# lawfuyang/ToyRenderer

Hardware: AMD Instinct MI355X
Metric: Gmeshlets/s culled (whole node), 100M meshlets (higher is better)
Workload: dtype f32

## Files before the change

toyrenderer_amd/csrc/k_basepass_as.hip:

```cpp
#include <algorithm>
#include <cstdlib>
#include <string>
#include <type_traits>

#if defined(TR_STAMPS) || defined(TR_COUNT_SLOW) || defined(TR_COUNT_PATHS)
__device__ unsigned long long g_stampSums[8];
#define g_pathCount (g_stampSums + 4)
#endif
#include <atomic>
#include <memory>
#include <mutex>
#include <unordered_map>

#include "cull_math.hip.h"
#include "instance_cache.hip.h"
#include "meshlet_exact.hip.h"
#include "trhip_internal.h"

using namespace interop;

namespace
{

constexpr uint32_t kBlock = 256;
// ... 115 lines not shown
#ifdef TR_STAMPS
#define TR_STAMP(i) do { unsigned long long _t = __builtin_amdgcn_s_memtime(); __builtin_amdgcn_s_waitcnt(0xC07F); stampSum[i] += _t - stampLast; stampLast = _t; } while (0)
#else
#define TR_STAMP(i) do {} while (0)
#endif

#ifndef TR_LK_POLICY_ID
#define TR_LK_POLICY_ID 0
#endif
#if TR_LK_POLICY_ID == 0
#define TR_LK_POLICY ""
#elif TR_LK_POLICY_ID == 1
#define TR_LK_POLICY " sc0"
#elif TR_LK_POLICY_ID == 2
#define TR_LK_POLICY " sc1"
#elif TR_LK_POLICY_ID == 3
#define TR_LK_POLICY " sc0 sc1"
#elif TR_LK_POLICY_ID == 4
#define TR_LK_POLICY " nt"
#else
#define TR_LK_POLICY " sc1 nt"
#endif
#ifndef TR_CULL_WAVES_PER_EU
#define TR_CULL_WAVES_PER_EU 5
#endif
template <bool FRUSTUM, bool OCCLUSION, bool CONE, bool TABLE>
__global__ __launch_bounds__(kCullBlock, TR_CULL_WAVES_PER_EU) void meshletCullKernel(MeshletCullArgs a)
{
#ifdef TR_STAMPS
    unsigned long long stampSum[8] = {0, 0, 0, 0, 0, 0, 0, 0};
    unsigned long long stampLast = __builtin_amdgcn_s_memtime();
    __builtin_amdgcn_s_waitcnt(0xC07F);
#endif
    __shared__ RecordInfo s_recAll[kCullWaves][kCullBatch + 2 * kRingSlots];
    __shared__ uint32_t s_gIdxAll[kCullWaves][kCullBatch];
    __shared__ uint32_t s_quadOff[16];
    __shared__ uint4 s_mipTab[17];
    __shared__ float s_coneTab[cm::kConeTabEntries];
    constexpr bool kDeferred = OCCLUSION && TABLE;
    __shared__ uint2 s_mipBand[kDeferred ? 17 : 1];
    __shared__ uint32_t s_defAll[kCullWaves][kDeferred ? kDefStage * kDefWords : 1u];
    __shared__ __attribute__((aligned(8))) uint32_t s_maskAll[kCullWaves][kCullBatch + 2];
    __shared__ __attribute__((aligned(16))) char s_ring[kCullWaves][kRingSlots][kSlotBytes];

    const uint32_t G = groupCount(a);
    const uint32_t tid = threadIdx.x, lane = tid & 63u, wave = tid >> 6;
    const uint32_t half = lane >> 5, sub = lane & 31u;
    if (a.listGroups && blockIdx.x == 0 && tid == 0) a.listGroups[0] = G;
    const cm::M43 V = cm::loadM43(a.k.m_WorldToView);
    const cm::M43P VP = cm::packM43(V);
    const cm::M33P VR = cm::rot(VP);
    const float coneSlack = cm::coneSlackFactor(V);
    if (!TABLE && G <= gridDim.x * (2u * kCullWaves) * a.shortPassRounds) {
        for (uint32_t g = (blockIdx.x * kCullWaves + wave) * 2u + half; g < G; g += gridDim.x * kCullWaves * 2u) {
            const bool vis = exactMeshletVisible<FRUSTUM, OCCLUSION, CONE>(a, VP, VR, g, sub);
            const unsigned long long b = __ballot(vis);
            if (sub == 0) a.visMask[g] = (uint32_t)(half ? b >> 32 : b);
        }
        return;
    }
    RecordInfo* s_rec = s_recAll[wave];
    uint32_t* s_gIdx = s_gIdxAll[wave];

    if (tid < 16) s_quadOff[tid] = a.hzb.mipOffset[tid];
    if (TABLE && tid >= 1 && tid <= 16) {
        const uint32_t mip = tid - 1u < a.hzb.mips ? tid - 1u : 0u;
        const uint32_t mw = (a.hzb.width >> mip) ? (a.hzb.width >> mip) : 1u, mh = (a.hzb.height >> mip) ? (a.hzb.height >> mip) : 1u;
        s_mipTab[tid] = make_uint4(a.quad.offset[mip], ((mw >> 3) + 1u) * 64u, __float_as_uint(0.5f * (float)mw), __float_as_uint(0.5f * (float)mh));
    }
    if (kDeferred && tid >= 1 && tid <= 16) { const uint32_t d = cm::projMipDelta(a.bands, tid); s_mipBand[tid] = make_uint2(d, 2u * d); }
    const bool nearInRange = a.k.m_NearPlane >= 0x1p-20f && a.k.m_NearPlane <= 0x1p20f;
    if (CONE) for (uint32_t i = tid; i < cm::kConeTabEntries; i += kCullBlock) s_coneTab[i] = cm::coneTableEntry(i);
    if (lane < 2 * kRingSlots) { s_recAll[wave][kCullBatch + lane].first = 0; s_recAll[wave][kCullBatch + lane].lastOff = 0; }
    uint32_t* s_def = s_defAll[wave];
    uint32_t* s_mask = s_maskAll[wave];
    __syncthreads();

    const bool usePerm = a.permHeader != nullptr && a.permHeader[0] == 1u && a.permHeader[1] == G;
#ifndef TR_TEAM_ALL
    const uint32_t teamWaves = kCullWaves, waveInTeam = wave, team = blockIdx.x, teams = gridDim.x;
#else
    const uint32_t teamWaves = gridDim.x * kCullWaves, waveInTeam = blockIdx.x * kCullWaves + wave, team = 0u, teams = 1u;
#endif
    const uint32_t superSize = teamWaves * kCullBatch;
    const uint32_t numSuper = (G + superSize - 1) / superSize;
    auto loadEntry = [&](uint32_t sb_) -> uint4 {
#ifdef TR_BLOCKED_MAP
        const uint64_t e64 = (uint64_t)sb_ * superSize + waveInTeam * kCullBatch + lane;
#else
        const uint64_t e64 = (uint64_t)sb_ * superSize + (lane >> 1) * 2 * teamWaves + 2 * waveInTeam + (lane & 1);
#endif
        if (lane >= kCullBatch || sb_ >= numSuper || e64 >= G) return make_uint4(0xFFFFFFFFu, 0u, 0u, 0u);
        const uint32_t e = (uint32_t)e64;
        if (usePerm) return a.perm[e];
        const MeshletAmplificationData rec = a.records[e];
        return make_uint4(e, rec.m_InstanceConstIdx, rec.m_MeshLOD, rec.m_MeshletGroupOffset);
    };
#ifndef TR_NO_SPLIT_TAIL
    const uint32_t fullRounds = numSuper / teams, left = numSuper - fullRounds * teams;
    uint32_t piecesPer = 1u, stepsPer = kCullSteps;
    if (left) {
        const uint32_t k = std::min(teams / left, kCullSteps / kRingSlots);
        if (k > 1u) {
            stepsPer = ((kCullSteps + k - 1u) / k + kRingSlots - 1u) / kRingSlots * kRingSlots;
            piecesPer = (kCullSteps + stepsPer - 1u) / stepsPer;
        }
// ... 1003 lines not shown
    }
    if (rc != TRHIP_OK) return rc;
    a.meshlets = (const MeshletData*)meshlets->ptr;
    TRHIP_REQUIRE(meshlets->byteSize >= sizeof(MeshletData), "%s: empty meshlet buffer", ctx.shaderName);
    rc = meshlets->cullStream.allocate(meshlets->dev, meshletStreamBytes(meshlets->byteSize / sizeof(MeshletData)));
    if (rc != TRHIP_OK) return rc;
    a.stream = meshletStreamLayout(meshlets->cullStream.ptr, meshlets->byteSize / sizeof(MeshletData));
    a.records = (const MeshletAmplificationData*)records->ptr;
    a.dispatchArgs = (const uint32_t*)((const char*)ctx.argsBuffer->ptr + ctx.argsOffset);
    a.argsWords = (ctx.argsBuffer->byteSize - ctx.argsOffset) >= 16 ? 4u : 3u;
    const uint64_t cap = records->byteSize / sizeof(MeshletAmplificationData);
    a.recordCapacity = cap > 0xFFFFFFFFull ? 0xFFFFFFFFu : (uint32_t)cap;
    TRHIP_REQUIRE(a.recordCapacity <= (1u << 27), "%s: more than 2^27 records cannot be encoded as (g<<5)|lane", ctx.shaderName);
    TRHIP_REQUIRE(visMask->byteSize / 4 >= a.recordCapacity, "%s: visMask holds %llu groups, records buffer %u", ctx.shaderName,
                  (unsigned long long)(visMask->byteSize / 4), a.recordCapacity);
    a.numMeshlets = meshlets->byteSize / sizeof(MeshletData);
    TRHIP_REQUIRE(a.numMeshlets <= (1ull << 32), "%s: more than 2^32 meshlets (m_MeshletDataBufferIdx is 32 bits wide)", ctx.shaderName);
    a.visMask = (uint32_t*)visMask->ptr;
    a.visibleList = (uint32_t*)visList->ptr;
    const uint64_t lcap = visList->byteSize / 4;
    a.listCapacity = lcap > 0xFFFFFFFFull ? 0xFFFFFFFFu : (uint32_t)lcap;
    a.drawArgs = (uint32_t*)drawArgs->ptr;
    if (records->order.ptr && records->order.bytes >= 256 + (uint64_t)a.recordCapacity * 16) {
        a.permHeader = (const uint32_t*)records->order.ptr;
        a.perm = (const uint4*)(a.permHeader + 64);
    }
    rc = trhip::instanceCacheEnsure(instances);
    if (rc != TRHIP_OK) return rc;
    a.numInstances = (uint32_t)(instances->byteSize / sizeof(BasePassInstanceConstants));
    a.cache = instanceCacheLayout(instances->cullCache.ptr, a.numInstances);
    a.maxBatches = (a.recordCapacity + kBatch - 1) / kBatch;
    a.batchSum = (uint32_t*)(a.recordCapacity >= (1u << 19) ? ctx.scratchSide((size_t)a.maxBatches * 4)
                                                            : ctx.scratch((size_t)a.maxBatches * 4));
    TRHIP_REQUIRE(a.batchSum, "%s: scratch allocation failed", ctx.shaderName);
    {
        const size_t supers = (a.maxBatches >> kSuperShift) + 1u;
        a.superSum = (uint32_t*)(a.recordCapacity >= (1u << 19) ? ctx.scratchSide(supers * 4) : ctx.scratch(supers * 4));
        TRHIP_REQUIRE(a.superSum, "%s: scratch allocation failed", ctx.shaderName);
    }

    const uint32_t blocksPerCU = TR_CULL_WAVES_PER_EU;
    uint32_t grid = ctx.computeUnits() * blocksPerCU;
    const uint32_t needBlocks = (a.recordCapacity + kCullBatch * kCullWaves - 1) / (kCullBatch * kCullWaves);
    if (grid > needBlocks) grid = needBlocks;
    if (grid == 0) grid = 1;
    rc = visMask->listCount.allocate(visMask->dev, 256);
    if (rc != TRHIP_OK) return rc;
    a.listGroups = (uint32_t*)visMask->listCount.ptr;
    ctx.cl->use(a.listGroups, ctx.cl->ops.size(), true);
    if (useTable) a.bands = cm::projBands(k->m_P00, k->m_P11, hzb->width, hzb->height);
    static const bool noShortPass = getenv("TRHIP_NO_SHORT_PASS") != nullptr;
    a.shortPassRounds = noShortPass ? 0u : kShortPassRounds;
    const uint32_t flags = k->m_CullingFlags & 7u;
    trhip_texture_t* quadOwner = useTable ? hzb : nullptr;
    const bool table = useTable;
    if (quadOwner) ctx.cl->use(quadOwner->quad.ptr, ctx.cl->ops.size(), false);
    ctx.emit("cull", [a, grid, flags, quadOwner, table, instances, meshData, meshlets](hipStream_t s) {
        if ((const void*)a.meshlets != meshlets->ptr)
            return trhip::fail(TRHIP_ERR_STATE, "basepass_AS_Main: the meshlet buffer was bound to other memory after this command list was recorded: record it again");
        {
            int crc = trhip::instanceCacheLaunchBuild(instances, meshData, s);
            if (crc != TRHIP_OK) return crc;
            crc = meshletStreamLaunchBuild(meshlets, s);
            if (crc != TRHIP_OK) return crc;
        }
        if (quadOwner) {
            int brc = trhip::hzbQuadLaunchBuild(quadOwner, s);
            if (brc != TRHIP_OK) return brc;
        }
        switch (flags) {
        case 0: launchCull<false, false, false>(a, grid, table, s); break;
        case 1: launchCull<true, false, false>(a, grid, table, s); break;
        case 2: launchCull<false, true, false>(a, grid, table, s); break;
        case 3: launchCull<true, true, false>(a, grid, table, s); break;
        case 4: launchCull<false, false, true>(a, grid, table, s); break;
        case 5: launchCull<true, false, true>(a, grid, table, s); break;
        case 6: launchCull<false, true, true>(a, grid, table, s); break;
        default: launchCull<true, true, true>(a, grid, table, s); break;
        }
        return trhip::launchStatus("meshletCullKernel"); });
    emitListBuild(ctx, a, "", a.recordCapacity >= (1u << 19), ctx.argsBuffer->ptr);
    if (ctx.cl->openStats)
        return trhip::statsEmitAS(ctx, a, meshlets, records, instances, meshData, a.recordCapacity >= (1u << 19));
    return TRHIP_OK;
}

int recordPackShard(trhip::DispatchCtx& ctx)
{
    const uint32_t* push = (const uint32_t*)ctx.constants(0, 8);
    trhip_buffer_t* slot = ctx.buffer(TRHIP_BIND_STRUCTURED_UAV, 0);
    trhip_buffer_t* state = ctx.buffer(TRHIP_BIND_STRUCTURED_UAV, 1);
    TRHIP_REQUIRE(push && slot && state, "%s: needs push constants {slotGroups, slotRuns}, UAV u0 (shard slot) and UAV u1 (state words, zeroed once)", ctx.shaderName);
    ShardPackArgs a;
    memset(&a, 0, sizeof a);
    a.slotGroups = push[0];
    a.slotRuns = push[1];
    const uint64_t slotWords = (uint64_t)kSlotHeaderWords + 4ull * a.slotRuns + a.slotGroups;
    TRHIP_REQUIRE(slot->byteSize >= slotWords * 4, "%s: shard slot buffer smaller than 16 + 4 * %u + %u words", ctx.shaderName, a.slotRuns, a.slotGroups);
    const uint64_t maxTiles = (uint64_t)a.slotGroups / kPackTile + kMaxPassSlots + 1u;
    TRHIP_REQUIRE(maxTiles < (1u << 30) && state->byteSize >= maxTiles * 16u, "%s: state buffer u1 smaller than %llu bytes", ctx.shaderName, (unsigned long long)(maxTiles * 16u));
    TRHIP_REQUIRE(((uintptr_t)slot->ptr & 15u) == 0 && ((uintptr_t)state->ptr & 7u) == 0, "%s: u0 / u1 not 16 / 8-byte aligned", ctx.shaderName);
    a.slot = (uint32_t*)slot->ptr;
    a.maxTiles = (uint32_t)maxTiles;
    unsigned long long* halves = (unsigned long long*)state->ptr;
    for (uint32_t s = 0; s < kMaxPassSlots; ++s) {
        trhip_buffer_t* rec = ctx.buffer(TRHIP_BIND_STRUCTURED_SRV, 4 * s);
// ... 122 lines not shown
```

toyrenderer_amd/csrc/k_gpuculling.hip:

```cpp
#include "cull_math.hip.h"
#include "hzb_quad.hip.h"
#include "instance_cache.hip.h"
#include "trhip_internal.h"

using namespace interop;

namespace
{

constexpr uint32_t kBlock = 256;
constexpr uint32_t kWordSubmit = 1u << 30;
constexpr uint32_t kWordLate = 1u << 31;
constexpr uint32_t kGroupMask = (1u << 27) - 1u;

struct InstanceCullArgs
{
    GPUCullingPassConstants k;
    const BasePassInstanceConstants* instances;
    const uint32_t* ids;
    const MeshData* meshData;
    cm::Hzb hzb;
    MeshletAmplificationData* records;
    uint32_t* dispatchArgs;
    uint32_t* lateCount;
    uint32_t* lateIds;
    const uint32_t* indirectArgs;
    InstanceCullCache cache;
    uint32_t numInstances;
    const uint32_t* shardLate;
    uint32_t directThreads;
    uint32_t maxGroups;
    uint32_t argsWords;
    uint32_t* word;
    uint32_t* localOff;
    uint32_t* blockGroups;
    uint64_t* blockLateSubmit;
    uint32_t* bases;
    uint32_t numBlocks;
    uint32_t* tileHist;
    uint32_t* tileTotal;
    uint16_t* tileOf;
    uint2* lodSel;
    uint32_t* permHeader;
    uint4* perm;
    uint32_t permCapacity;
    uint32_t* lateArgsOut;
    unsigned long long* fusedStatus;
    uint32_t* fusedTicket;
};

struct QuadShare { bool stale = false; };
struct EarlyCullNote { InstanceCullArgs a; size_t scanOp; bool fused; trhip_texture_t* quadOwner = nullptr; std::shared_ptr<QuadShare> share; };

__global__ __launch_bounds__(256) void instanceCacheKernel(const BasePassInstanceConstants* instances, uint32_t n,
                                                           const MeshData* meshData, uint32_t numMeshes, InstanceCullCache c)
// ... 367 lines not shown
        const bool emitRec = submit && !dropped;
        const uint32_t id = emitRec ? a.ids[t] : 0u;
        if (emitRec) {
            struct __attribute__((packed, aligned(4))) Quad { uint32_t x, y, z, w; };
            uint32_t* dst = reinterpret_cast<uint32_t*>(a.records + off);
            uint32_t i = 0;
            for (; i + 4u <= groups; i += 4u) {
                const uint32_t o = i * kNumThreadsPerWave;
                *reinterpret_cast<Quad*>(dst + 3u * i) = Quad{ id, lod, o, id };
                *reinterpret_cast<Quad*>(dst + 3u * i + 4u) = Quad{ lod, o + kNumThreadsPerWave, id, lod };
                *reinterpret_cast<Quad*>(dst + 3u * i + 8u) = Quad{ o + 2u * kNumThreadsPerWave, id, lod, o + 3u * kNumThreadsPerWave };
            }
            for (; i < groups; ++i) {
                MeshletAmplificationData rec = { id, lod, i * kNumThreadsPerWave };
                a.records[off + i] = rec;
            }
        }
        const bool place = emitRec && groups != 0 && binned;
        uint32_t p = 0, numMeshlets = 0, mbase = 0;
        if (place) {
            p = atomicAdd(&s_cursor[a.tileOf[t]], groups);
            const uint2 li = a.lodSel[t];
            numMeshlets = li.x; mbase = li.y;
        }
        const uint32_t head = place ? (groups < 4u ? groups : 4u) : 0u;
        const uint32_t j = lane & 3u;
#pragma unroll
        for (uint32_t it = 0; it < 4; ++it) {
            const int src = (int)(it * 16u + (lane >> 2));
            const uint32_t sp = __shfl(p, src), soff = __shfl(off, src), sid = __shfl(id, src);
            const uint32_t sbase = __shfl(mbase, src), snm = __shfl(numMeshlets, src), shead = __shfl(head, src);
            if (j < shead) {
                const uint32_t first = j * kNumThreadsPerWave;
                const uint32_t cnt = snm > first ? (snm - first < kNumThreadsPerWave ? snm - first : kNumThreadsPerWave) : 0u;
                if (sp + j < a.permCapacity) a.perm[sp + j] = make_uint4(soff + j, sid, sbase + first, cnt);
            }
        }
        if (place)
            for (uint32_t i = 4; i < groups; ++i) {
                const uint32_t first = i * kNumThreadsPerWave;
                const uint32_t cnt = numMeshlets > first ? (numMeshlets - first < kNumThreadsPerWave ? numMeshlets - first : kNumThreadsPerWave) : 0u;
                if (p + i < a.permCapacity) a.perm[p + i] = make_uint4(off + i, id, mbase + first, cnt);
            }
    }
}


constexpr uint32_t kFusedMaxEntries = 1u << 17;
constexpr uint32_t kFusedMaxTiles = kFusedMaxEntries / kBlock;
constexpr uint32_t kFusedLateMaxTiles = 4096;
constexpr uint32_t kFusedStatusStride = 16;
constexpr unsigned long long kFusedFlag = 1ull << 63, kFusedPoison = 1ull << 60;

template <int LATE>
__global__ __launch_bounds__(kBlock) void instanceFusedKernel(InstanceCullArgs a, trhip::QuadArgs q)
{
    if (!LATE && blockIdx.x >= a.numBlocks) {
        __shared__ float s_t[9][trhip::kQuadStripCols + 1];
        trhip::hzbQuadStrip(q, blockIdx.x - a.numBlocks, s_t);
        return;
    }
    __shared__ uint32_t s_waveG[kBlock / 64], s_waveL[kBlock / 64], s_waveS[kBlock / 64];
    __shared__ unsigned long long s_preG[kBlock / 64], s_preLS[kBlock / 64];
    __shared__ uint32_t s_tile;
    const uint32_t n = threadCount<LATE>(a);
    const uint32_t numTiles = (n + kBlock - 1) / kBlock < a.numBlocks ? (n + kBlock - 1) / kBlock : a.numBlocks;
    const uint32_t tid = threadIdx.x, lane = tid & 63u, wave = tid >> 6;
    const uint32_t baseX = __hip_atomic_load(&a.dispatchArgs[0], __ATOMIC_RELAXED, __HIP_MEMORY_SCOPE_AGENT);
    const uint32_t baseLate = LATE ? 0u : __hip_atomic_load(a.lateCount, __ATOMIC_RELAXED, __HIP_MEMORY_SCOPE_AGENT);
    if (blockIdx.x >= (numTiles ? numTiles : 1u)) return;
    {
        if (tid == 0) s_tile = atomicAdd(a.fusedTicket, 1u);
        __syncthreads();
        const uint32_t tile = s_tile;
        const uint32_t t = tile * kBlock + tid;
        uint32_t word = 0, tileUnused = 0;
        uint2 lodUnused;
        if (t < n) word = classify<LATE>(a, a.ids[t], &tileUnused, &lodUnused);
        const uint32_t g = (word & kWordSubmit) ? (word & kGroupMask) : 0u;
        const uint32_t late = word >> 31;
        const uint32_t submit = (word >> 30) & 1u;
        const uint32_t incG = waveInclusiveScan(g, lane);
        const uint32_t incL = waveInclusiveScan(late, lane);
        const uint32_t cntS = (uint32_t)__popcll(__ballot(submit != 0));
        if (lane == 63) { s_waveG[wave] = incG; s_waveL[wave] = incL; s_waveS[wave] = cntS; }
        __syncthreads();
        uint32_t baseG = 0, baseL = 0, totG = 0, totL = 0, totS = 0;
#pragma unroll
        for (uint32_t w = 0; w < kBlock / 64; ++w) {
            if (w < wave) { baseG += s_waveG[w]; baseL += s_waveL[w]; }
            totG += s_waveG[w]; totL += s_waveL[w]; totS += s_waveS[w];
        }
        const uint32_t localOff = late ? (baseL + incL - late) : (baseG + incG - g);
        unsigned long long* line = a.fusedStatus + (uint64_t)tile * kFusedStatusStride;
        if (tid == 0 && numTiles != 0) {
            __hip_atomic_store(&line[0], kFusedFlag | (unsigned long long)totG, __ATOMIC_RELAXED, __HIP_MEMORY_SCOPE_AGENT);
            __hip_atomic_store(&line[1], kFusedFlag | ((unsigned long long)totS << 32) | (unsigned long long)totL, __ATOMIC_RELAXED, __HIP_MEMORY_SCOPE_AGENT);
        }
        unsigned long long sumG = 0, sumLS = 0;
        for (uint32_t j = tid; j < tile; j += kBlock) {
            const unsigned long long* pl = a.fusedStatus + (uint64_t)j * kFusedStatusStride;
            unsigned long long v0 = 0, v1 = 0;
            uint32_t spins = 0;
            for (;;) {
                v0 = __hip_atomic_load(&pl[0], __ATOMIC_RELAXED, __HIP_MEMORY_SCOPE_AGENT);
                v1 = __hip_atomic_load(&pl[1], __ATOMIC_RELAXED, __HIP_MEMORY_SCOPE_AGENT);
                if ((v0 & v1 & kFusedFlag) != 0ull) { v0 &= ~kFusedFlag; v1 &= ~kFusedFlag; break; }
                if (++spins > (1u << 22)) { v0 = kFusedPoison; v1 = 0; break; }
                __builtin_amdgcn_s_sleep(1);
            }
            sumG += v0; sumLS += v1;
        }
#pragma unroll
        for (int d = 32; d >= 1; d >>= 1) { sumG += __shfl_xor(sumG, d); sumLS += __shfl_xor(sumLS, d); }
        if (lane == 0) { s_preG[wave] = sumG; s_preLS[wave] = sumLS; }
        __syncthreads();
        unsigned long long preG = 0, preLS = 0;
#pragma unroll
        for (uint32_t w = 0; w < kBlock / 64; ++w) { preG += s_preG[w]; preLS += s_preLS[w]; }
        const uint32_t prefixG = (uint32_t)preG, prefixL = (uint32_t)preLS;
        if (t < n) {
            if (word & kWordLate) {
                a.lateIds[baseLate + prefixL + localOff] = a.ids[t];
            } else if (word & kWordSubmit) {
                const uint32_t groups = word & kGroupMask;
                const uint32_t lod = (word >> 27) & 7u;
                const uint32_t off = baseX + prefixG + localOff;
                if (off + groups >= a.maxGroups) {
                    if (groups != 0 && off < a.maxGroups && a.argsWords > 3) a.dispatchArgs[3] = off;
                } else {
                    const uint32_t id = a.ids[t];
                    for (uint32_t i = 0; i < groups; ++i) {
                        MeshletAmplificationData rec = { id, lod, i * kNumThreadsPerWave };
                        a.records[off + i] = rec;
                    }
                }
            }
        }
        if (tid == 0 && (tile == numTiles - 1u || numTiles == 0)) {
            const unsigned long long allG = preG + totG;
            const uint32_t allL = prefixL + totL, allS = (uint32_t)(preLS >> 32) + totS;
            const uint32_t X = (allG >> 40) ? 0xFFFFFFFFu : baseX + (uint32_t)allG;
            a.bases[0] = baseX;
            a.bases[1] = baseLate;
            a.dispatchArgs[0] = X;
            if (allS != 0) { a.dispatchArgs[1] = 1; a.dispatchArgs[2] = 1; }
            if (a.argsWords > 3 && (X < a.maxGroups || baseX >= a.maxGroups)) a.dispatchArgs[3] = X;
            if (!LATE) {
                const uint32_t lateTotal = baseLate + allL;
                *a.lateCount = lateTotal;
                if (a.lateArgsOut) { a.lateArgsOut[0] = (lateTotal + 63u) / 64u; a.lateArgsOut[1] = 1; a.lateArgsOut[2] = 1; }
            }
            a.permHeader[0] = 0u;
            a.permHeader[1] = X;
        }
    }
}

__global__ void buildLateCullIndirectArgsKernel(const uint32_t* count, uint32_t* args)
{
    args[0] = (count[0] + 63u) / 64u;
    args[1] = 1;
    args[2] = 1;
}

__global__ void shardLateInfoKernel(const uint32_t* counts, uint32_t world, uint32_t rank, uint32_t* info)
{
    uint32_t below = 0, all = 0;
    for (uint32_t p = 0; p < world; ++p) {
        const uint32_t c = counts[p];
        if (p < rank) below += c;
        all += c;
    }
    info[0] = below;
    info[1] = all;
}

int fillHzb(const trhip::DispatchCtx& ctx, trhip_texture_t* tex, const Vector2U& dims, bool occlusion, cm::Hzb* out)
{
    memset(out, 0, sizeof *out);
    if (!occlusion) return TRHIP_OK;
    TRHIP_REQUIRE(tex, "%s: occlusion culling enabled but no HZB texture bound", ctx.shaderName);
    TRHIP_REQUIRE(tex->format == TRHIP_FORMAT_R16_FLOAT, "%s: HZB '%s' is not R16_FLOAT", ctx.shaderName, tex->name.c_str());
    TRHIP_REQUIRE(tex->width == dims.x && tex->height == dims.y,
                  "%s: m_HZBDimensions %ux%u does not match HZB texture %ux%u", ctx.shaderName, dims.x, dims.y, tex->width, tex->height);
    out->base = (const _Float16*)tex->ptr;
    out->width = tex->width; out->height = tex->height; out->mips = tex->mips;
    for (uint32_t k = 0; k < tex->mips; ++k) out->mipOffset[k] = (uint32_t)(tex->mipOffset[k] / 2);
    return TRHIP_OK;
}

std::function<int(hipStream_t)> fusedEarlyLaunch(const InstanceCullArgs& a, trhip_texture_t* quadOwner)
{
    return [a, quadOwner](hipStream_t s) {
        trhip::QuadArgs q;
        memset(&q, 0, sizeof q);
        uint32_t strips = 0;
        if (quadOwner && !quadOwner->quad.current({ quadOwner->version })) {
            q = trhip::quadArgs(quadOwner);
            strips = q.firstStrip[q.mips];
            quadOwner->quad.markBuilt({ quadOwner->version });
        }
        TRHIP_LAUNCH(instanceFusedKernel<0>, dim3(a.numBlocks + strips), dim3(kBlock), 0, s, a, q);
        return trhip::launchStatus("instanceFusedKernel"); };
}

inline uint32_t quadScanStrips(uint32_t all)
{
    static const uint32_t pct = [] { const char* e = getenv("TRHIP_QUAD_SCAN_PERCENT"); const int v = e ? atoi(e) : 50; return (uint32_t)(v < 0 ? 0 : v > 100 ? 100 : v); }();
    return (uint32_t)((uint64_t)all * pct / 100u);
}

std::function<int(hipStream_t)> scanEarlyLaunch(const InstanceCullArgs& a, trhip_texture_t* quadOwner, std::shared_ptr<QuadShare> share)
{
    return [a, quadOwner, share](hipStream_t s) {
        trhip::QuadArgs q;
        memset(&q, 0, sizeof q);
        uint32_t extra = 0, stripEnd = 0;
        if (share) share->stale = false;
        if (quadOwner && !quadOwner->quad.current({ quadOwner->version })) {
            q = trhip::quadArgs(quadOwner);
            stripEnd = share ? quadScanStrips(q.firstStrip[q.mips]) : q.firstStrip[q.mips];
            extra = (stripEnd + kScanStripsPerGroup - 1u) / kScanStripsPerGroup;
            quadOwner->quad.markBuilt({ quadOwner->version });
            if (share) share->stale = true;
        }
        TRHIP_LAUNCH(instanceScanKernel<0>, dim3(1 + kScanTileGroups + extra), dim3(kScanThreads), 0, s, a, q, stripEnd);
        return trhip::launchStatus("instanceScanKernel"); };
}

template <int LATE>
int recordGPUCulling(trhip::DispatchCtx& ctx)
{
    const GPUCullingPassConstants* k = (const GPUCullingPassConstants*)ctx.constants(0, sizeof(GPUCullingPassConstants));
    TRHIP_REQUIRE(k, "%s: constant buffer b0 (GPUCullingPassConstants, 180 bytes) missing", ctx.shaderName);
    trhip_buffer_t* instances = ctx.buffer(TRHIP_BIND_STRUCTURED_SRV, 0);
    trhip_buffer_t* ids = ctx.buffer(TRHIP_BIND_STRUCTURED_SRV, 1);
    trhip_buffer_t* meshData = ctx.buffer(TRHIP_BIND_STRUCTURED_SRV, 2);
    trhip_texture_t* hzb = ctx.texture(TRHIP_BIND_TEXTURE_SRV, 3);
    trhip_buffer_t* records = ctx.buffer(TRHIP_BIND_STRUCTURED_UAV, 0);
    trhip_buffer_t* args = ctx.buffer(TRHIP_BIND_STRUCTURED_UAV, 1);
    trhip_buffer_t* lateCount = ctx.buffer(TRHIP_BIND_STRUCTURED_UAV, 2);
    trhip_buffer_t* lateIds = ctx.buffer(TRHIP_BIND_STRUCTURED_UAV, 3);
    trhip_buffer_t* shardLate = LATE ? ctx.buffer(TRHIP_BIND_STRUCTURED_SRV, 4) : nullptr;
    TRHIP_REQUIRE(!shardLate || shardLate->byteSize >= 8, "%s: shard late info (t4) smaller than 8 bytes", ctx.shaderName);
    TRHIP_REQUIRE(instances && ids && meshData && records && args && lateCount && lateIds,
                  "%s: needs SRVs t0..t2 and UAVs u0..u3 (BasePassRenderers.cpp:351-362)", ctx.shaderName);
    const bool occlusion = (k->m_CullingFlags & kCullingFlagOcclusionCullingEnable) != 0;
    TRHIP_REQUIRE(instances->byteSize % sizeof(BasePassInstanceConstants) == 0, "%s: instance buffer size is not a multiple of 144", ctx.shaderName);
    TRHIP_REQUIRE(meshData->byteSize % sizeof(MeshData) == 0, "%s: mesh data buffer size is not a multiple of 156", ctx.shaderName);
    TRHIP_REQUIRE(records->byteSize >= sizeof(MeshletAmplificationData), "%s: amplification buffer too small", ctx.shaderName);
    TRHIP_REQUIRE(args->byteSize >= 12, "%s: dispatch-arguments buffer smaller than 12 bytes", ctx.shaderName);
    if (LATE) {
        TRHIP_REQUIRE(ctx.indirect, "%s: LATE_CULL=1 is dispatched indirectly (BasePassRenderers.cpp:399)", ctx.shaderName);
        TRHIP_REQUIRE(occlusion, "%s: LATE_CULL=1 without occlusion culling", ctx.shaderName);
        TRHIP_REQUIRE((uint64_t)k->m_NbInstances * 4 <= lateIds->byteSize, "%s: late id buffer smaller than m_NbInstances", ctx.shaderName);
    } else {
// ... 16 lines not shown
    a.dispatchArgs = (uint32_t*)args->ptr;
    a.lateCount = (uint32_t*)lateCount->ptr;
    a.lateIds = (uint32_t*)lateIds->ptr;
    a.indirectArgs = LATE ? (const uint32_t*)((const char*)ctx.argsBuffer->ptr + ctx.argsOffset) : nullptr;
    a.shardLate = shardLate ? (const uint32_t*)shardLate->ptr : nullptr;
    const uint64_t direct = (uint64_t)ctx.gx * kNumThreadsPerWave;
    a.directThreads = direct > 0xFFFFFFFFull ? 0xFFFFFFFFu : (uint32_t)direct;
    const uint64_t cap = records->byteSize / sizeof(MeshletAmplificationData);
    a.maxGroups = cap > 0xFFFFFFFFull ? 0xFFFFFFFFu : (uint32_t)cap;
    a.argsWords = args->byteSize >= 16 ? 4u : 3u;

    const uint32_t nMax = k->m_NbInstances;
    if (nMax == 0) return TRHIP_OK;

    rc = trhip::instanceCacheEnsure(instances);
    if (rc != TRHIP_OK) return rc;
    a.cache = instanceCacheLayout(instances->cullCache.ptr, instances->byteSize / sizeof(BasePassInstanceConstants));
    a.numInstances = (uint32_t)(instances->byteSize / sizeof(BasePassInstanceConstants));
    ctx.emit("instance_cache", [instances, meshData](hipStream_t s) { return trhip::instanceCacheLaunchBuild(instances, meshData, s); });
    static const bool noFused = getenv("TRHIP_NO_FUSED_INSTANCE") != nullptr;
    const bool fusedPath = (nMax <= kFusedMaxEntries || (LATE && (nMax + kBlock - 1) / kBlock <= kFusedLateMaxTiles)) && !noFused;
    a.numBlocks = fusedPath ? (nMax + kBlock - 1) / kBlock : (nMax + kBigChunk - 1) / kBigChunk;
    a.word = (uint32_t*)ctx.scratch((size_t)nMax * 4);
    a.localOff = (uint32_t*)ctx.scratch((size_t)nMax * 4);
    a.blockGroups = (uint32_t*)ctx.scratch((size_t)a.numBlocks * 4);
    a.blockLateSubmit = (uint64_t*)ctx.scratch((size_t)a.numBlocks * 8);
    a.bases = (uint32_t*)ctx.scratch(16);
    a.tileHist = (uint32_t*)ctx.scratch(fusedPath ? 16 : (size_t)a.numBlocks * kNumTiles * 4);
    a.tileTotal = (uint32_t*)ctx.scratch(kNumTiles * 4);
    a.tileOf = (uint16_t*)ctx.scratch((size_t)nMax * 2);
    a.lodSel = (uint2*)ctx.scratch((size_t)nMax * 8);
    TRHIP_REQUIRE(a.word && a.localOff && a.blockGroups && a.blockLateSubmit && a.bases && a.tileHist && a.tileTotal && a.tileOf && a.lodSel, "%s: scratch allocation failed", ctx.shaderName);
    rc = records->order.allocate(records->dev, (uint64_t)kPermHeaderWords * 4 + (uint64_t)a.maxGroups * 16);
    if (rc != TRHIP_OK) return rc;
    a.permHeader = (uint32_t*)records->order.ptr;
    a.perm = (uint4*)(a.permHeader + kPermHeaderWords);
    a.permCapacity = a.maxGroups;
    const bool wantTable = !LATE && occlusion && a.maxGroups >= trhip::tableMinGroups();
    if (wantTable) {
        rc = trhip::hzbQuadEnsure(hzb);
        if (rc != TRHIP_OK) return rc;
    }

    if (fusedPath) {
        const size_t words = (size_t)a.numBlocks * kFusedStatusStride * 2 + 4;
        uint32_t* mem = (uint32_t*)ctx.scratch(words * 4);
        TRHIP_REQUIRE(mem, "%s: scratch allocation failed", ctx.shaderName);
        rc = ctx.cl->recordClearWords(mem, words, 0, true);
        if (rc != TRHIP_OK) return rc;
        a.fusedStatus = (unsigned long long*)mem;
        a.fusedTicket = mem + (size_t)a.numBlocks * kFusedStatusStride * 2;
        trhip_texture_t* quadOwner = wantTable ? hzb : nullptr;
        if (quadOwner) ctx.cl->use(quadOwner->quad.ptr, ctx.cl->ops.size(), true);
        if (LATE) ctx.emit("fused", [a](hipStream_t s) {
            trhip::QuadArgs q;
            memset(&q, 0, sizeof q);
            TRHIP_LAUNCH(instanceFusedKernel<LATE>, dim3(a.numBlocks), dim3(kBlock), 0, s, a, q);
            return trhip::launchStatus("instanceFusedKernel"); });
        else ctx.emit("fused", fusedEarlyLaunch(a, quadOwner));
        if (!LATE && occlusion) ctx.cl->peephole = { ctx.cl->ops.size() - 1, "gpuculling_early", std::make_shared<EarlyCullNote>(EarlyCullNote{ a, ctx.cl->ops.size() - 1, true, quadOwner }) };
        return TRHIP_OK;
    }

    ctx.emit("classify", [a](hipStream_t s) {
        TRHIP_LAUNCH(instanceClassifyKernel<LATE>, dim3(a.numBlocks), dim3(kBigThreads), 0, s, a);
        return trhip::launchStatus("instanceClassifyKernel"); });
    trhip_texture_t* quadOwner = wantTable ? hzb : nullptr;
    std::shared_ptr<QuadShare> share = quadOwner ? std::make_shared<QuadShare>() : nullptr;
    if (quadOwner) ctx.cl->use(quadOwner->quad.ptr, ctx.cl->ops.size(), true);
    if (LATE) ctx.emit("scan", [a](hipStream_t s) {
        trhip::QuadArgs q;
        memset(&q, 0, sizeof q);
        TRHIP_LAUNCH(instanceScanKernel<LATE>, dim3(1 + kScanTileGroups), dim3(kScanThreads), 0, s, a, q, 0u);
        return trhip::launchStatus("instanceScanKernel"); });
    else ctx.emit("scan", scanEarlyLaunch(a, quadOwner, share));
    const size_t scanOp = ctx.cl->ops.size() - 1;
    if (quadOwner) ctx.cl->use(quadOwner->quad.ptr, ctx.cl->ops.size(), true);
    ctx.emit("emit", [a, quadOwner, share](hipStream_t s) {
        trhip::QuadArgs q;
        memset(&q, 0, sizeof q);
        uint32_t extra = 0, stripBegin = 0;
        if (!LATE && quadOwner && share && share->stale) {
            q = trhip::quadArgs(quadOwner);
            stripBegin = quadScanStrips(q.firstStrip[q.mips]);
            extra = (q.firstStrip[q.mips] - stripBegin + kEmitStripsPerGroup - 1u) / kEmitStripsPerGroup;
        }
        TRHIP_LAUNCH(instanceEmitKernel<LATE>, dim3(a.numBlocks + extra), dim3(kBigThreads), 0, s, a, q, stripBegin);
        return trhip::launchStatus("instanceEmitKernel"); });
    if (!LATE && occlusion) ctx.cl->peephole = { ctx.cl->ops.size() - 1, "gpuculling_early", std::make_shared<EarlyCullNote>(EarlyCullNote{ a, scanOp, false, quadOwner, share }) };
    return TRHIP_OK;
}

int recordBuildLateArgs(trhip::DispatchCtx& ctx)
{
    trhip_buffer_t* count = ctx.buffer(TRHIP_BIND_STRUCTURED_SRV, 0);
    trhip_buffer_t* args = ctx.buffer(TRHIP_BIND_STRUCTURED_UAV, 0);
    TRHIP_REQUIRE(count && args, "%s: needs SRV t0 (late count) and UAV u0 (indirect args)", ctx.shaderName);
    TRHIP_REQUIRE(count->byteSize >= 4 && args->byteSize >= 12, "%s: buffers too small", ctx.shaderName);
    TRHIP_REQUIRE(!ctx.indirect && ctx.gx == 1 && ctx.gy == 1 && ctx.gz == 1, "%s: dispatched as 1x1x1", ctx.shaderName);
    const uint32_t* c = (const uint32_t*)count->ptr;
    uint32_t* a = (uint32_t*)args->ptr;
    const trhip_cmdlist_t::Peephole ph = ctx.cl->peephole;
    if (ph.kind && !strcmp(ph.kind, "gpuculling_early") && ph.op != SIZE_MAX && ph.op == ctx.cl->ops.size() - 1) {
        const EarlyCullNote* note = (const EarlyCullNote*)ph.data.get();
        if (note->a.lateCount == c && note->scanOp < ctx.cl->ops.size() && ctx.cl->ops[note->scanOp].lane == 0) {
            InstanceCullArgs fused = note->a;
            fused.lateArgsOut = a;
            const size_t scanOp = note->scanOp;
            if (note->fused) ctx.cl->ops[scanOp].fn = fusedEarlyLaunch(fused, note->quadOwner);
            else ctx.cl->ops[scanOp].fn = scanEarlyLaunch(fused, note->quadOwner, note->share);
            for (size_t i = ctx.cl->useMarks.size(); i-- > 0 && ctx.cl->useMarks[i].op >= ctx.cl->ops.size();) ctx.cl->useMarks[i].op = scanOp;
// ... 49 lines not shown
```

toyrenderer_amd/csrc/meshlet_exact.hip.h:

```cpp
#pragma once

#include <hip/hip_runtime.h>

#include "ShaderInterop.h"
#include "cull_math.hip.h"
#include "instance_cache.hip.h"

using namespace interop;

struct MeshletCullStream
{
    const float4* sphere;
    const uint32_t* cone;
};

struct MeshletCullArgs
{
    BasePassConstants k;
    const MeshletData* meshlets;
    MeshletCullStream stream;
    const MeshletAmplificationData* records;
    cm::Hzb hzb;
    cm::HzbQuad quad;
    const uint32_t* dispatchArgs;
    uint32_t argsWords;
    uint32_t recordCapacity;
    uint64_t numMeshlets;
    uint32_t* visMask;
    uint32_t* visibleList; uint32_t listCapacity;
    uint32_t* drawArgs;
    uint32_t* batchSum;
    uint32_t* superSum;
    uint32_t maxBatches;
    const uint32_t* permHeader;
    const uint4* perm;
    InstanceCullCache cache;
    uint32_t numInstances;
    uint32_t* listGroups;
    cm::ProjBands bands;
    uint32_t shortPassRounds;
};

__device__ __forceinline__ uint32_t groupCount(const MeshletCullArgs& a)
{
    uint32_t G = a.dispatchArgs[0];
    if (a.argsWords > 3 && a.dispatchArgs[3] < G) G = a.dispatchArgs[3];
    return G < a.recordCapacity ? G : a.recordCapacity;
}

template <bool FRUSTUM, bool OCCLUSION, bool CONE>
__device__ __forceinline__ bool exactMeshletAt(const MeshletCullArgs& a, const cm::M43P& VP, const cm::M33P& VR, uint32_t cid, uint64_t mi)
{
    const float4* wr = a.cache.world + 4ull * cid;
    const float4* p = reinterpret_cast<const float4*>(a.meshlets + mi);
    const float4 q0 = wr[0], q1 = wr[1], q2 = wr[2], q3 = wr[3];
    const float4 sphere = p[0];
    const uint32_t cone = __float_as_uint(p[1].x);
    const cm::F3 r0 = { q0.x, q0.y, q0.z }, r1 = { q0.w, q1.x, q1.y }, r2 = { q1.z, q1.w, q2.x };
    const cm::M43P W = cm::packM43(cm::M43{ r0, r1, r2, { q2.y, q2.z, q2.w } });
    const cm::M33P adj = cm::rot(cm::packM43(cm::M43{ cm::cross3(r1, r2), cm::cross3(r2, r0), cm::cross3(r0, r1), { 0.f, 0.f, 0.f } }));
    const cm::F3 cv = cm::toViewP(cm::mulPointP({ sphere.x, sphere.y, sphere.z }, W), VP);
    const float rad = sphere.w * q3.x;
    bool vis = true;
    if (FRUSTUM) vis &= cm::frustumVisible(cv, rad, a.k.m_Frustum.x, a.k.m_Frustum.y, a.k.m_Frustum.z, a.k.m_Frustum.w);
    if (OCCLUSION) vis &= cm::occlusionVisible(cv, rad, a.k.m_NearPlane, a.k.m_P00, a.k.m_P11, a.hzb);
    float unused;
    if (CONE) vis &= !cm::coneBackfacingP(cone, cv, rad, adj, VR, 1.0f, 1.0f, &unused);
    return vis;
}
template <bool FRUSTUM, bool OCCLUSION, bool CONE>
__device__ __forceinline__ bool exactMeshletVisible(const MeshletCullArgs& a, const cm::M43P& VP, const cm::M33P& VR, uint32_t g, uint32_t m)
{
    const MeshletAmplificationData rec = a.records[g];
    const uint32_t cid = rec.m_InstanceConstIdx < a.numInstances ? rec.m_InstanceConstIdx : 0u;
    const uint32_t lodIdx = rec.m_MeshLOD < kMaxNumMeshLODs ? rec.m_MeshLOD : kMaxNumMeshLODs - 1u;
    const uint2 li = a.cache.lod(cid, lodIdx);
    const uint32_t off = rec.m_MeshletGroupOffset;
    uint32_t cnt = li.x > off ? li.x - off : 0u;
    const uint64_t base = (uint64_t)li.y + off;
    cnt = cnt < 32u ? cnt : 32u;
    if (base + cnt > a.numMeshlets) cnt = 0;
    if (m >= cnt) return false;
    return exactMeshletAt<FRUSTUM, OCCLUSION, CONE>(a, VP, VR, cid, base + m);
}
```

toyrenderer_amd/csrc/trhip_core.cpp:

```cpp
#include "trhip_internal.h"
#include "r11g11b10.hip.h"

#include <chrono>
#include <cmath>
#include <cstdlib>

#include <algorithm>
#include <memory>

namespace trhip
{

static thread_local char tl_error[1024] = "";

int fail(int code, const char* fmt, ...)
{
    va_list ap;
    va_start(ap, fmt);
    vsnprintf(tl_error, sizeof tl_error, fmt, ap);
    va_end(ap);
    return code;
}

int hipfail(hipError_t e, const char* what)
// ... 226 lines not shown
            if (grid > (uint64_t)cus * 8u) grid = (uint64_t)cus * 8u;
            if (grid == 0) grid = 1;
            TRHIP_LAUNCH(multiClearKernel, dim3((uint32_t)grid), dim3(256), 0, s, a);
            return trhip::launchStatus("multiClearKernel"); } });
        ops.back().kind = "clear_buffer";
        openClearOp = ops.size() - 1;
        if (!firstClearBatch) { firstClearBatch = openClearBatch; firstClearOp = openClearOp; }
    }
    ClearBatch& b = *openClearBatch;
    b.ptr[b.count] = ptr; b.words[b.count] = words; b.value[b.count] = value;
    ++b.count;
    return TRHIP_OK;
}

void trhip_cmdlist_t::hold(trhip_buffer_t* b, bool write, size_t op) { if (b) { use(b->ptr, op == SIZE_MAX ? ops.size() : op, write, &b->version); trhip_buffer_retain(b); heldBuffers.push_back(b); } }
void trhip_cmdlist_t::hold(trhip_texture_t* t, bool write) { if (t) { use(t->ptr, ops.size(), write, &t->version); trhip_texture_retain(t); heldTextures.push_back(t); } }

extern "C" {

const char* trhip_last_error(void) { return tl_error; }
uint32_t trhip_abi_version(void) { return TRHIP_ABI_VERSION; }
uint32_t trhip_shader_count(void) { return (uint32_t)shaders().size(); }
const char* trhip_shader_name(uint32_t i) { return i < shaders().size() ? shaders()[i].name.c_str() : nullptr; }
int trhip_shader_exists(const char* name) { return name && findShader(name) ? 1 : 0; }

static int deviceCreate(int index, void* stream, bool external, trhip_device* out)
{
    if (!out) return fail(TRHIP_ERR_INVALID, "out is null");
    int n = 0;
    if (hipGetDeviceCount(&n) != hipSuccess || n <= 0)
        return fail(TRHIP_ERR_NO_DEVICE, "no HIP device visible (this back end has no CPU fallback)");
    if (index < 0 || index >= n) return fail(TRHIP_ERR_INVALID, "device index %d out of range (%d devices)", index, n);
    TRHIP_HIP(hipSetDevice(index));
    hipDeviceProp_t props;
    TRHIP_HIP(hipGetDeviceProperties(&props, index));
    auto dev = std::make_unique<trhip_device_t>();
    dev->index = index;
    dev->computeUnits = (uint32_t)props.multiProcessorCount;
    dev->waveSize = (uint32_t)props.warpSize;
    dev->totalMem = (uint64_t)props.totalGlobalMem;
    if (dev->waveSize != 64)
        return fail(TRHIP_ERR_INVALID, "wave size %u: the kernels are written for wave64 (gfx950)", dev->waveSize);
    if (external) {
        dev->stream = (hipStream_t)stream;
        dev->ownsStream = false;
    } else {
        TRHIP_HIP(hipStreamCreateWithFlags(&dev->stream, hipStreamNonBlocking));
        dev->ownsStream = true;
    }
    if (!getenv("TRHIP_NO_SIDE_STREAM")) {
        int lowest = 0, highest = 0;
        TRHIP_HIP(hipDeviceGetStreamPriorityRange(&lowest, &highest));
        TRHIP_HIP(hipStreamCreateWithPriority(&dev->sideStream, hipStreamNonBlocking, highest));
        TRHIP_HIP(hipEventCreateWithFlags(&dev->evFork, hipEventDisableTiming));
        for (hipEvent_t& e : dev->runDone) TRHIP_HIP(hipEventCreateWithFlags(&e, hipEventDisableTiming));
    }
    *out = dev.release();
    return TRHIP_OK;
}

int trhip_device_create(int device_index, trhip_device* out) { return deviceCreate(device_index, nullptr, false, out); }
int trhip_device_create_on_stream(int device_index, void* s, trhip_device* out) { return deviceCreate(device_index, s, true, out); }

void trhip_device_destroy(trhip_device dev)
{
    if (!dev) return;
    (void)hipSetDevice(dev->index);
    (void)dev->syncAll();
    (void)dev->drainProfile();
    for (hipEvent_t e : dev->eventPool) (void)hipEventDestroy(e);
    if (dev->sideStream) { (void)hipStreamSynchronize(dev->sideStream); (void)hipStreamDestroy(dev->sideStream); }
    if (dev->evFork) (void)hipEventDestroy(dev->evFork);
    for (hipEvent_t e : dev->runDone) if (e) (void)hipEventDestroy(e);
    if (dev->ownsStream) (void)hipStreamDestroy(dev->stream);
    delete dev;
}

int trhip_device_wait_idle(trhip_device dev)
{
    if (!dev) return fail(TRHIP_ERR_INVALID, "device is null");
    TRHIP_HIP(hipSetDevice(dev->index));
    return dev->syncAll();
}

int trhip_device_join_side_stream(trhip_device dev)
{
    if (!dev) return fail(TRHIP_ERR_INVALID, "device is null");
    TRHIP_HIP(hipSetDevice(dev->index));
    std::lock_guard<std::mutex> lock(dev->mutex);
    if (dev->sideStream && dev->sideRunCounter > dev->mainWaitedUpTo) {
        TRHIP_HIP(hipStreamWaitEvent(dev->stream, dev->runDone[dev->sideRunCounter % trhip_device_t::kSideRuns], 0));
        dev->mainWaitedUpTo = dev->sideRunCounter;
    }
    return TRHIP_OK;
}

int trhip_device_info(trhip_device dev, uint32_t* cus, uint32_t* wave, uint64_t* mem)
{
    if (!dev) return fail(TRHIP_ERR_INVALID, "device is null");
    if (cus) *cus = dev->computeUnits;
    if (wave) *wave = dev->waveSize;
    if (mem) *mem = dev->totalMem;
    return TRHIP_OK;
}

void* trhip_device_stream(trhip_device dev) { return dev ? (void*)dev->stream : nullptr; }

int trhip_heap_create(trhip_device dev, uint64_t bytes, trhip_heap* out)
// ... 811 lines not shown
```

toyrenderer_amd/csrc/trhip_internal.h:

```cpp
#pragma once

#include <hip/hip_runtime.h>

#include <atomic>
#include <cstdarg>
#include <cstdint>
#include <cstdio>
#include <cstdlib>
#include <cstring>
#include <functional>
#include <map>
#include <memory>
#include <mutex>
#include <string>
#include <unordered_map>
#include <vector>

#include <hip/hip_ext.h>

#include "../../include/trhip.h"
#include "ShaderInterop.h"

namespace trhip
{
// ... 206 lines not shown
    }

    struct Peephole { size_t op = SIZE_MAX; const char* kind = nullptr; std::shared_ptr<void> data; } peephole;

    void* scratchAlloc(size_t bytes);
    void* scratchAllocSide(size_t bytes);
    std::vector<ScratchBlock> sideScratch;
    void resetRecording();
    void hold(trhip_buffer_t* b, bool write, size_t op = SIZE_MAX);
    void hold(trhip_texture_t* t, bool write);
};

namespace trhip
{

struct DispatchCtx
{
    trhip_cmdlist_t* cl;
    const char* shaderName;
    int variant;
    const trhip_binding* bindings; uint32_t numBindings;
    const void* push; uint32_t pushBytes;
    bool indirect; trhip_buffer_t* argsBuffer; uint32_t argsOffset;
    uint32_t gx, gy, gz;

    trhip_buffer_t* buffer(uint32_t type, uint32_t slot) const;
    trhip_texture_t* texture(uint32_t type, uint32_t slot, uint32_t* baseMip = nullptr) const;
    const void* constants(uint32_t slot, size_t bytes) const;
    uint32_t computeUnits() const { return cl->dev->computeUnits; }
    void* scratch(size_t bytes) const { return cl->scratchAlloc(bytes); }
    void* scratchSide(size_t bytes) const { return cl->dev->sideStream ? cl->scratchAllocSide(bytes) : cl->scratchAlloc(bytes); }
    void emit(const char* kernelName, std::function<int(hipStream_t)> fn) const;
    void emitSide(const char* kernelName, std::function<int(hipStream_t)> fn, std::initializer_list<Op::Access> touched) const;
};

int hzbQuadEnsure(trhip_texture_t* tex);
int hzbQuadLaunchBuild(trhip_texture_t* tex, hipStream_t s);

int instanceCacheEnsure(trhip_buffer_t* instances);
int instanceCacheLaunchBuild(trhip_buffer_t* instances, trhip_buffer_t* meshData, hipStream_t s);

inline uint32_t tableMinGroups()
{
    static const uint32_t v = [] { const char* e = getenv("TRHIP_TABLE_MIN_GROUPS"); return e ? (uint32_t)strtoul(e, nullptr, 0) : (1u << 17); }();
    return v;
}

uint32_t statsCSThreads(const char* shaderName);
int statsLaunchAdd(unsigned long long* counter, uint64_t value, hipStream_t s);
int statsEmitIndirectCS(trhip_cmdlist_t* cl, trhip_buffer_t* args, uint32_t argsOffset, uint32_t threads);
int statsEmitAS(const DispatchCtx& ctx, const ::MeshletCullArgs& a, trhip_buffer_t* meshlets, trhip_buffer_t* records,
                trhip_buffer_t* instances, trhip_buffer_t* meshData, bool side);

using RecordFn = int (*)(DispatchCtx&);
void registerShader(const char* name, RecordFn fn, int variant);

struct ShaderRegistrar
{
    ShaderRegistrar(const char* name, RecordFn fn, int variant = 0) { registerShader(name, fn, variant); }
};

struct LaunchTap { hipStream_t onStream = nullptr; hipEvent_t stopEvent = nullptr; int launches = 0; };
extern thread_local LaunchTap* g_launchTap;
#define TRHIP_LAUNCH(kernel, grid, block, shmem, stream, ...)                                                       \
    do {                                                                                                            \
        trhip::LaunchTap* tap_ = trhip::g_launchTap;                                                                \
        if (tap_ && tap_->onStream == (stream) && ++tap_->launches)                                              \
            hipExtLaunchKernelGGL(kernel, grid, block, shmem, stream, nullptr, tap_->stopEvent, 0, __VA_ARGS__);    \
        else                                                                                                        \
            hipLaunchKernelGGL(kernel, grid, block, shmem, stream, __VA_ARGS__);                                    \
    } while (0)

inline int launchStatus(const char* what)
{
    hipError_t e = hipGetLastError();
    return e == hipSuccess ? TRHIP_OK : hipfail(e, what);
}

}
```

Before: 122.0.

## Fuse late meshlet culling into late instance-cull kernel via command-list peephole

```diff
diff --git a/toyrenderer_amd/csrc/k_basepass_as.hip b/toyrenderer_amd/csrc/k_basepass_as.hip
--- a/toyrenderer_amd/csrc/k_basepass_as.hip
+++ b/toyrenderer_amd/csrc/k_basepass_as.hip
@@ -191,6 +191,7 @@
     const cm::M33P VR = cm::rot(VP);
     const float coneSlack = cm::coneSlackFactor(V);
     if (!TABLE && G <= gridDim.x * (2u * kCullWaves) * a.shortPassRounds) {
+        if (a.inlineDone && *a.inlineDone != 0u) return;
         for (uint32_t g = (blockIdx.x * kCullWaves + wave) * 2u + half; g < G; g += gridDim.x * kCullWaves * 2u) {
             const bool vis = exactMeshletVisible<FRUSTUM, OCCLUSION, CONE>(a, VP, VR, g, sub);
             const unsigned long long b = __ballot(vis);
@@ -1300,6 +1301,20 @@
     static const bool noShortPass = getenv("TRHIP_NO_SHORT_PASS") != nullptr;
     a.shortPassRounds = noShortPass ? 0u : kShortPassRounds;
     const uint32_t flags = k->m_CullingFlags & 7u;
+    static const bool noInlineLate = getenv("TRHIP_NO_INLINE_LATE_CULL") != nullptr;
+    const trhip_cmdlist_t::Peephole ph = ctx.cl->peephole;
+    if (ctx.variant == 1 && !useTable && !noInlineLate && ph.kind && !strcmp(ph.kind, "gpuculling_late") && ph.op != SIZE_MAX &&
+        ph.op == ctx.cl->ops.size() - 1 && ctx.cl->ops[ph.op].lane == 0) {
+        const trhip::LateCullNote* note = (const trhip::LateCullNote*)ph.data.get();
+        const uint32_t limit = grid * (2u * kCullWaves) * a.shortPassRounds;
+        if (limit != 0 && note->records == (const void*)a.records && note->dispatchArgs == (const void*)a.dispatchArgs && note->argsWords == a.argsWords &&
+            note->recordCapacity == a.recordCapacity && note->instanceCache == instances->cullCache.ptr) {
+            a.inlineDone = note->inlineDone;
+            note->install(a, limit, flags, meshlets);
+            for (size_t i = ctx.cl->useMarks.size(); i-- > 0 && ctx.cl->useMarks[i].op > ph.op;) ctx.cl->useMarks[i].op = ph.op;
+        }
+    }
+    ctx.cl->peephole = trhip_cmdlist_t::Peephole();
     trhip_texture_t* quadOwner = useTable ? hzb : nullptr;
     const bool table = useTable;
     if (quadOwner) ctx.cl->use(quadOwner->quad.ptr, ctx.cl->ops.size(), false);
diff --git a/toyrenderer_amd/csrc/k_gpuculling.hip b/toyrenderer_amd/csrc/k_gpuculling.hip
--- a/toyrenderer_amd/csrc/k_gpuculling.hip
+++ b/toyrenderer_amd/csrc/k_gpuculling.hip
@@ -1,6 +1,7 @@
 #include "cull_math.hip.h"
 #include "hzb_quad.hip.h"
 #include "instance_cache.hip.h"
+#include "meshlet_exact.hip.h"
 #include "trhip_internal.h"
 
 using namespace interop;
@@ -474,23 +475,23 @@
 constexpr uint32_t kFusedStatusStride = 16;
 constexpr unsigned long long kFusedFlag = 1ull << 63, kFusedPoison = 1ull << 60;
 
-template <int LATE>
-__global__ __launch_bounds__(kBlock) void instanceFusedKernel(InstanceCullArgs a, trhip::QuadArgs q)
+template <int LATE, bool RANGE>
+__device__ __forceinline__ bool fusedPass(const InstanceCullArgs& a, const trhip::QuadArgs& q, uint32_t* inlineDone, uint32_t* recBegin, uint32_t* recEnd)
 {
     if (!LATE && blockIdx.x >= a.numBlocks) {
         __shared__ float s_t[9][trhip::kQuadStripCols + 1];
         trhip::hzbQuadStrip(q, blockIdx.x - a.numBlocks, s_t);
-        return;
+        return false;
     }
     __shared__ uint32_t s_waveG[kBlock / 64], s_waveL[kBlock / 64], s_waveS[kBlock / 64];
     __shared__ unsigned long long s_preG[kBlock / 64], s_preLS[kBlock / 64];
-    __shared__ uint32_t s_tile;
+    __shared__ uint32_t s_tile, s_recEnd;
     const uint32_t n = threadCount<LATE>(a);
     const uint32_t numTiles = (n + kBlock - 1) / kBlock < a.numBlocks ? (n + kBlock - 1) / kBlock : a.numBlocks;
     const uint32_t tid = threadIdx.x, lane = tid & 63u, wave = tid >> 6;
     const uint32_t baseX = __hip_atomic_load(&a.dispatchArgs[0], __ATOMIC_RELAXED, __HIP_MEMORY_SCOPE_AGENT);
     const uint32_t baseLate = LATE ? 0u : __hip_atomic_load(a.lateCount, __ATOMIC_RELAXED, __HIP_MEMORY_SCOPE_AGENT);
-    if (blockIdx.x >= (numTiles ? numTiles : 1u)) return;
+    if (blockIdx.x >= (numTiles ? numTiles : 1u)) return false;
     {
         if (tid == 0) s_tile = atomicAdd(a.fusedTicket, 1u);
         __syncthreads();
@@ -541,6 +542,10 @@
 #pragma unroll
         for (uint32_t w = 0; w < kBlock / 64; ++w) { preG += s_preG[w]; preLS += s_preLS[w]; }
         const uint32_t prefixG = (uint32_t)preG, prefixL = (uint32_t)preLS;
+        if (RANGE) {
+            if (tid == 0) s_recEnd = baseX + prefixG + totG;
+            __syncthreads();
+        }
         if (t < n) {
             if (word & kWordLate) {
                 a.lateIds[baseLate + prefixL + localOff] = a.ids[t];
@@ -550,6 +555,7 @@
                 const uint32_t off = baseX + prefixG + localOff;
                 if (off + groups >= a.maxGroups) {
                     if (groups != 0 && off < a.maxGroups && a.argsWords > 3) a.dispatchArgs[3] = off;
+                    if (RANGE && groups != 0) atomicMin(&s_recEnd, off);
                 } else {
                     const uint32_t id = a.ids[t];
                     for (uint32_t i = 0; i < groups; ++i) {
@@ -575,9 +581,41 @@
             }
             a.permHeader[0] = 0u;
             a.permHeader[1] = X;
-        }
-    }
-}
+            if (RANGE && baseX == 0) *inlineDone = 1u;
+        }
+        if (RANGE) {
+            __syncthreads();
+            *recBegin = baseX + prefixG;
+            *recEnd = baseX == 0 ? s_recEnd : *recBegin;
+        }
+    }
+    return true;
+}
+
+template <int LATE>
+__global__ __launch_bounds__(kBlock) void instanceFusedKernel(InstanceCullArgs a, trhip::QuadArgs q)
+{
+    fusedPass<LATE, false>(a, q, nullptr, nullptr, nullptr);
+}
+
+template <bool FRUSTUM, bool OCCLUSION, bool CONE>
+__global__ __launch_bounds__(kBlock) void instanceFusedLateCullKernel(InstanceCullArgs a, MeshletCullArgs m, uint32_t limit, uint32_t* inlineDone)
+{
+    const trhip::QuadArgs q = {};
+    uint32_t recBegin = 0, recEnd = 0;
+    if (!fusedPass<1, true>(a, q, inlineDone, &recBegin, &recEnd)) return;
+    const cm::M43P VP = cm::packM43(cm::loadM43(m.k.m_WorldToView));
+    const cm::M33P VR = cm::rot(VP);
+    const uint32_t lane = threadIdx.x & 63u, wave = threadIdx.x >> 6;
+    const uint32_t half = lane >> 5, sub = lane & 31u;
+    const uint32_t end = recEnd < limit ? recEnd : limit;
+    for (uint32_t g = recBegin + wave * 2u + half; g < end; g += (kBlock / 64u) * 2u) {
+        const bool vis = exactMeshletVisible<FRUSTUM, OCCLUSION, CONE>(m, VP, VR, g, sub);
+        const unsigned long long b = __ballot(vis);
+        if (sub == 0) m.visMask[g] = (uint32_t)(half ? b >> 32 : b);
+    }
+}
+
 
 __global__ void buildLateCullIndirectArgsKernel(const uint32_t* count, uint32_t* args)
 {
@@ -625,6 +663,39 @@
         }
         TRHIP_LAUNCH(instanceFusedKernel<0>, dim3(a.numBlocks + strips), dim3(kBlock), 0, s, a, q);
         return trhip::launchStatus("instanceFusedKernel"); };
+}
+
+std::function<int(hipStream_t)> fusedLateLaunch(const InstanceCullArgs& a)
+{
+    return [a](hipStream_t s) {
+        trhip::QuadArgs q;
+        memset(&q, 0, sizeof q);
+        TRHIP_LAUNCH(instanceFusedKernel<1>, dim3(a.numBlocks), dim3(kBlock), 0, s, a, q);
+        return trhip::launchStatus("instanceFusedKernel"); };
+}
+
+template <bool F, bool O, bool C>
+void launchFusedLateCull(const InstanceCullArgs& a, const MeshletCullArgs& m, uint32_t limit, uint32_t* inlineDone, hipStream_t s)
+{
+    TRHIP_LAUNCH((instanceFusedLateCullKernel<F, O, C>), dim3(a.numBlocks), dim3(kBlock), 0, s, a, m, limit, inlineDone);
+}
+
+std::function<int(hipStream_t)> fusedLateCullLaunch(const InstanceCullArgs& a, const MeshletCullArgs& m, uint32_t limit, uint32_t flags,
+                                                    uint32_t* inlineDone, const trhip_buffer_t* meshlets)
+{
+    return [a, m, limit, flags, inlineDone, meshlets, plain = fusedLateLaunch(a)](hipStream_t s) {
+        if ((const void*)m.meshlets != meshlets->ptr) return plain(s);
+        switch (flags & 7u) {
+        case 0: launchFusedLateCull<false, false, false>(a, m, limit, inlineDone, s); break;
+        case 1: launchFusedLateCull<true, false, false>(a, m, limit, inlineDone, s); break;
+        case 2: launchFusedLateCull<false, true, false>(a, m, limit, inlineDone, s); break;
+        case 3: launchFusedLateCull<true, true, false>(a, m, limit, inlineDone, s); break;
+        case 4: launchFusedLateCull<false, false, true>(a, m, limit, inlineDone, s); break;
+        case 5: launchFusedLateCull<true, false, true>(a, m, limit, inlineDone, s); break;
+        case 6: launchFusedLateCull<false, true, true>(a, m, limit, inlineDone, s); break;
+        default: launchFusedLateCull<true, true, true>(a, m, limit, inlineDone, s); break;
+        }
+        return trhip::launchStatus("instanceFusedLateCullKernel"); };
 }
 
 inline uint32_t quadScanStrips(uint32_t all)
@@ -747,11 +818,18 @@
         a.fusedTicket = mem + (size_t)a.numBlocks * kFusedStatusStride * 2;
         trhip_texture_t* quadOwner = wantTable ? hzb : nullptr;
         if (quadOwner) ctx.cl->use(quadOwner->quad.ptr, ctx.cl->ops.size(), true);
-        if (LATE) ctx.emit("fused", [a](hipStream_t s) {
-            trhip::QuadArgs q;
-            memset(&q, 0, sizeof q);
-            TRHIP_LAUNCH(instanceFusedKernel<LATE>, dim3(a.numBlocks), dim3(kBlock), 0, s, a, q);
-            return trhip::launchStatus("instanceFusedKernel"); });
+        if (LATE) {
+            ctx.emit("fused", fusedLateLaunch(a));
+            trhip_cmdlist_t* cl = ctx.cl;
+            const size_t op = cl->ops.size() - 1;
+            uint32_t* inlineDone = a.fusedTicket + 1;
+            auto note = std::make_shared<trhip::LateCullNote>();
+            note->records = a.records; note->dispatchArgs = a.dispatchArgs; note->argsWords = a.argsWords; note->recordCapacity = a.maxGroups;
+            note->instanceCache = instances->cullCache.ptr; note->inlineDone = inlineDone;
+            note->install = [cl, op, a, inlineDone](const MeshletCullArgs& m, uint32_t limit, uint32_t flags, const trhip_buffer_t* meshlets) {
+                cl->ops[op].fn = fusedLateCullLaunch(a, m, limit, flags, inlineDone, meshlets); };
+            cl->peephole = { op, "gpuculling_late", note };
+        }
         else ctx.emit("fused", fusedEarlyLaunch(a, quadOwner));
         if (!LATE && occlusion) ctx.cl->peephole = { ctx.cl->ops.size() - 1, "gpuculling_early", std::make_shared<EarlyCullNote>(EarlyCullNote{ a, ctx.cl->ops.size() - 1, true, quadOwner }) };
         return TRHIP_OK;
diff --git a/toyrenderer_amd/csrc/meshlet_exact.hip.h b/toyrenderer_amd/csrc/meshlet_exact.hip.h
--- a/toyrenderer_amd/csrc/meshlet_exact.hip.h
+++ b/toyrenderer_amd/csrc/meshlet_exact.hip.h
@@ -39,6 +39,7 @@
     uint32_t* listGroups;
     cm::ProjBands bands;
     uint32_t shortPassRounds;
+    const uint32_t* inlineDone;
 };
 
 __device__ __forceinline__ uint32_t groupCount(const MeshletCullArgs& a)
diff --git a/toyrenderer_amd/csrc/trhip_core.cpp b/toyrenderer_amd/csrc/trhip_core.cpp
--- a/toyrenderer_amd/csrc/trhip_core.cpp
+++ b/toyrenderer_amd/csrc/trhip_core.cpp
@@ -302,8 +302,9 @@
         int lowest = 0, highest = 0;
         TRHIP_HIP(hipDeviceGetStreamPriorityRange(&lowest, &highest));
         TRHIP_HIP(hipStreamCreateWithPriority(&dev->sideStream, hipStreamNonBlocking, highest));
-        TRHIP_HIP(hipEventCreateWithFlags(&dev->evFork, hipEventDisableTiming));
-        for (hipEvent_t& e : dev->runDone) TRHIP_HIP(hipEventCreateWithFlags(&e, hipEventDisableTiming));
+        const unsigned forkFlags = hipEventDisableTiming | hipEventDisableSystemFence;
+        TRHIP_HIP(hipEventCreateWithFlags(&dev->evFork, forkFlags));
+        for (hipEvent_t& e : dev->runDone) TRHIP_HIP(hipEventCreateWithFlags(&e, forkFlags));
     }
     *out = dev.release();
     return TRHIP_OK;
diff --git a/toyrenderer_amd/csrc/trhip_internal.h b/toyrenderer_amd/csrc/trhip_internal.h
--- a/toyrenderer_amd/csrc/trhip_internal.h
+++ b/toyrenderer_amd/csrc/trhip_internal.h
@@ -282,6 +282,16 @@
 int statsEmitAS(const DispatchCtx& ctx, const ::MeshletCullArgs& a, trhip_buffer_t* meshlets, trhip_buffer_t* records,
                 trhip_buffer_t* instances, trhip_buffer_t* meshData, bool side);
 
+struct LateCullNote
+{
+    const void* records = nullptr;
+    const void* dispatchArgs = nullptr;
+    uint32_t argsWords = 0, recordCapacity = 0;
+    const void* instanceCache = nullptr;
+    uint32_t* inlineDone = nullptr;
+    std::function<void(const ::MeshletCullArgs& m, uint32_t limit, uint32_t flags, const trhip_buffer_t* meshlets)> install;
+};
+
 using RecordFn = int (*)(DispatchCtx&);
 void registerShader(const char* name, RecordFn fn, int variant);
 
```

After: 115.7. -5.2%, worse.
